# hezy18/SegMMInterest

Measured on AMD Instinct MI355X. Metric: train interactions/sec (segment-Transformer, B=512·S=40·D=768), higher is better.
Workload: dtype f32 (products via scaled fp16x2 split, 22-bit operands, fp32 accumulate; operands pre-split by their producers); 1 GPU; BASELINE config 2: synthetic SegMM B=512/GPU x S=40 x D_in=768 -> d=768, h=16, 2-layer segment encoder, image/image inputs, Lt=100 user tokens, interestBPR, dropout 0.1, AdamW; 8 distinct batches rotated; input=features; rows_per_gpu=512, global_batch=512, segments=40, feat_dim=768, in_dim=768, layers=2, parallelism=dp1, grad_allreduce_overlap=True, input_prefetch=False, delayed_scale_overflows=0, gemm_engine=f16x3p

## Files before the change

### segmminterest_amd/csrc/capi.hip

```cpp
#include <stdarg.h>
#include <stdio.h>
#include <string.h>
#include <stdlib.h>
#include <initializer_list>
#include <type_traits>

#include "../../include/segmm_hip.h"
#include "attention16.h"
#include "attention_pl.h"
#include "attention_stream.h"
#include "attention_wide.h"
#include "common.h"
#include "evalops.h"
#include "gemm.h"
#include "gemm_split.h"
#include "gemm_planes.h"
#include "gemm_planes8.h"
#include "gemm_planes4.h"
#include "loss.h"
#include "rowops.h"
#include "assemble.h"
#include "storeops.h"
#include "srops.h"

static int num_cus() {
    static int n = 0;
    if (n == 0) {
        int dev = 0;
        hipDeviceProp_t prop;
        if (hipGetDevice(&dev) == hipSuccess && hipGetDeviceProperties(&prop, dev) == hipSuccess) n = prop.multiProcessorCount;
        if (n <= 0) n = 256;
    }
    return n;
}
#ifdef SEGMM_STAMPS
static unsigned long long* g_segmm_stamps = nullptr;
extern "C" int segmm_debug_set_stamps(void* p) { g_segmm_stamps = (unsigned long long*)p; return 0; }
#endif

thread_local char g_segmm_err[512] = {0};

int segmm_fail(int code, const char* fmt, ...) {
    va_list ap;
    va_start(ap, fmt);
    vsnprintf(g_segmm_err, sizeof(g_segmm_err), fmt, ap);
    va_end(ap);
    return code;
}

#define LAUNCH_CHECK() SEGMM_CHECK_HIP(hipGetLastError())

StepState* g_segmm_step = nullptr;
static StepState* g_step_default = nullptr;
StepState* segmm_step_current() {
    if (g_segmm_step) return g_segmm_step;
    if (!g_step_default) {
        if (hipMalloc((void**)&g_step_default, sizeof(StepState)) != hipSuccess) return nullptr;
        (void)hipMemset(g_step_default, 0, sizeof(StepState));
    }
    return g_step_default;
}

using namespace segmm;

static inline int attn_keys_p(int La, int Lb) { return ((La + 15) & ~15) + ((Lb + 15) & ~15); }
static int attn_fill(AttnArgs& a, int B, int H, int dh, int Lq, int La, int Lb, const float* Qa, const float* Qb, int ldq,
                     const float* Ka, const float* Va, int ldka, const float* Kb, const float* Vb, int ldkb,
                     const uint8_t* mq, const uint8_t* mka, const uint8_t* mkb, float drop_p, uint64_t seed,
                     uint32_t site, bool planes_in = false) {
    SEGMM_REQUIRE(B > 0 && H > 0 && Lq > 0 && La >= 0 && Lb >= 0 && La + Lb > 0, "attn: empty dimension");
    if (La == 0) { Qa = Qb; Ka = Kb; Va = Vb; ldka = ldkb; mka = mkb; }
    if (Lb == 0) { Qb = Qa; Kb = Ka; Vb = Va; ldkb = ldka; mkb = mka; }
    SEGMM_REQUIRE(((Qa && Qb && Ka && Va && Kb && Vb) || (planes_in && !Qa && !Qb && !Ka && !Va && !Kb && !Vb)) && mq && mka && mkb, "attn: null pointer");
    SEGMM_REQUIRE(dh == 4 || dh == 8 || dh == 16 || dh == 32 || dh == 48 || dh == 64 || dh == 96 || dh == 128,
                  "attn: head dim %d not built (4,8,16,32,48,64,96,128)", dh);
    SEGMM_REQUIRE(!(planes_in && att_wide(dh)), "attn: input planes are not built for wide heads (head dim %d > 64): hand the fp32 views of Q / K / V", dh);
    SEGMM_REQUIRE(ldq % 4 == 0 && ldka % 4 == 0 && ldkb % 4 == 0, "attn: leading dims %% 4");
    SEGMM_REQUIRE(aligned16(Qa) && aligned16(Qb) && aligned16(Ka) && aligned16(Va) && aligned16(Kb) && aligned16(Vb), "attn: alignment");
    SEGMM_REQUIRE(Lq <= 256 && La <= 256 && Lb <= 256, "attn: Lq=%d, La=%d, Lb=%d not built (at most 256 queries and 256 keys per key block)", Lq, La, Lb);
    a.B = B; a.H = H; a.Lq = Lq; a.La = La; a.Lb = Lb;
    a.Qa = Qa; a.Qb = Qb; a.ldq = ldq; a.Ka = Ka; a.Va = Va; a.ldka = ldka; a.Kb = Kb; a.Vb = Vb; a.ldkb = ldkb;
    a.mq = mq; a.mka = mka; a.mkb = mkb;
    a.scale = 1.0f / sqrtf((float)dh);
    a.drop = make_drop(drop_p, seed, site);
    {
        const size_t ka = La ? ((size_t)B * La - 1) * ldka + (size_t)H * dh : 0, kb = Lb ? ((size_t)B * Lb - 1) * ldkb + (size_t)H * dh : 0;
        const size_t q = ((size_t)B * Lq - 1) * ldq + (size_t)H * dh;
        SEGMM_REQUIRE(((size_t)B * La + 16) * ldka * 4 < (1ull << 32) && ((size_t)B * Lb + 16) * ldkb * 4 < (1ull << 32) &&
                      ((size_t)B * Lq + 16) * ldq * 4 < (1ull << 32), "attn: a K/V/Q view exceeds the 4 GiB buffer-addressing window");
        a.ka_bytes = (uint32_t)(ka * 4); a.kb_bytes = (uint32_t)(kb * 4); a.q_bytes = (uint32_t)(q * 4);
    }
    return 0;
}

enum {
    K_ATTN, K_ATT_FWD_PL, K_ATT_FWD_LDS, K_ATT_FWD_KSPLIT, K_ATT_FWD_LDS_PAD, K_ATT_STREAM, K_ATT_FUSED_LAUNCH, K_ATT_MERGE, K_ATT_LDS_PAD, K_ATT_WAVES, K_ATT_WAVES_PL, K_ATT_REPAIR_WALK,
    K_ATT_HPB_FWD, K_ATT_HPB_DQ, K_ATT_HPB_DKV, K_L1NORM_REG, K_GEMM_BN, K_PL_VAR, K_PL_NJ, K_TN_VAR, K_LN_BWD_PARTS, K_DPRE_PLANES_ONLY, K_EMA_NT, K_LN_FWD_PARTS, K_COUNT
};
struct Knob { const char* name; int value; const char* doc; };
static Knob g_knobs[K_COUNT] = {
    {"ATTN", 1, "attention arithmetic: 0 (env: f32) exact-fp32 kernels only, 1 fp16x3 where measured faster, 2 (env: f16all) fp16x3 wherever built"},
    {"ATT_FWD_PL", 1, "planes-in forward when the caller hands input planes (0: never)"},
    {"ATT_FWD_LDS", 1, "LDS-DMA staged fp32 forward: 0 never, 1 heads with >= 4 query tiles, 2 wherever it fits"},
    {"ATT_FWD_KSPLIT", 1, "staged forward: key-tile groups per query tile"},
    {"ATT_FWD_LDS_PAD", 0, "probe: extra LDS bytes per forward workgroup (fewer workgroups per CU)"},
    {"ATT_STREAM", 0, "1: every fp32-view forward and every phase 0-3 backward through the streamed kernels (always taken above 192 padded keys)"},
    {"ATT_FUSED_LAUNCH", 2, "fused backward: 2 one launch per key block, 1 one launch for both"},
    {"ATT_MERGE", 1, "short heads: one workgroup per head for both key blocks in the fused backward"},
    {"ATT_LDS_PAD", 0, "probe: extra LDS bytes per backward workgroup"},
    {"ATT_WAVES", 4, "fused fp16x3 backward: waves per workgroup (key tiles in passes)"},
    {"ATT_WAVES_PL", 3, "planes-in fused backward: waves per workgroup, 1..4 (3: 40.7 KB of LDS -> four workgroups per CU for a 100-key block too)"},
    {"ATT_REPAIR_WALK", 512, "planes-in backward, repair launch: workgroups that walk the heads (0: one workgroup per head)"},
    {"ATT_HPB_FWD", 0, "forward workgroup shape heads | tiles << 8 (env: \"heads[,tiles]\"; 0: built-in)"},
    {"ATT_HPB_DQ", 0, "dQ kernel workgroup shape, as above"},
    {"ATT_HPB_DKV", 0, "dK/dV kernel workgroup shape, as above"},
    {"L1NORM_REG", 1, "L1 normalisation with the row held in registers"},
    {"GEMM_BN", 0, "on-the-fly GEMM: tile width override (0: built-in choice)"},
    {"PL_VAR", 4, "plane NT GEMM: 4 gemm_pl_nt4 (round 6: 128 x 256 tiles, two workgroups per CU) for K >= 768 and N >= 768, gemm_pl_nt8 otherwise; 44 gemm_pl_nt4 always; 8 gemm_pl_nt8 (round 3); 1: the round-2 fallback kernel for every launch"},
    {"PL_NJ", 0, "plane NT GEMM: tile width in 64-column units (0: modelled choice)"},
    {"TN_VAR", 8, "plane TN GEMM: 8 gemm_pl_tn4 (round 6: 128 x 256 tiles, two workgroups per CU) for few-tile and 128-row matrices, gemm_pl_tn8 (round 3) otherwise; 4 gemm_pl_tn4 wherever it fits; 88 gemm_pl_tn8 wherever it fits; 0: the round-2 fallback kernel for every launch"},
    {"LN_BWD_PARTS", 0, "LayerNorm backward: most workgroups (= partial rows of its column sums) per launch; 0: as many four-wave workgroups as are resident at the row width (768 at d = 768: one full round, no under-occupied tail)"},
    {"DPRE_PLANES_ONLY", 1, "embedding LayerNorm gradients as planes only + repair launch (no fp32 copy): 0 never, 1 for sites on the per-position grid today (rows * d >= 2^23), 2 wherever segmm_layernorm_bwd_pos_parts gives a grid (tests at small shapes), 3 as 1 for the user side only (A/B per site)"},
    {"EMA_NT", 0, "segmm_ema_update: 0 everything with the default cache policy, 1 the shadow loaded and stored nontemporally (p with the default policy); same bits (A/B: profiles/ema/)"},
    {"LN_FWD_PARTS", 0, "LayerNorm forward (d <= 1024): 0 one round of resident workgroups whose waves walk rows, grid by row width; 1 the one-wave-per-row form; 2 and up: that many workgroups in the walking form, clamped to 64..4096; same bits (A/B: profiles/row_stream/)"},
};
static bool g_knobs_ready = false;
static void knobs_init() {
    if (g_knobs_ready) return;
    g_knobs_ready = true;
    for (int k = 0; k < K_COUNT; ++k) {
        char name[64];
        snprintf(name, sizeof(name), "SEGMM_%s", g_knobs[k].name);
        const char* e = getenv(name);
        if (!e || !*e) continue;
        if (k == K_ATTN) g_knobs[k].value = !strcmp(e, "f32") ? 0 : !strcmp(e, "f16all") ? 2 : 1;
        else if (k == K_ATT_HPB_FWD || k == K_ATT_HPB_DQ || k == K_ATT_HPB_DKV) {
            const char* c = strchr(e, ',');
            g_knobs[k].value = (atoi(e) > 0 ? atoi(e) : 0) | ((c && atoi(c + 1) > 0 ? atoi(c + 1) : 0) << 8);
        } else g_knobs[k].value = atoi(e);
    }
}
static inline int knob(int k) { knobs_init(); return g_knobs[k].value; }
int segmm_config_set(const char* name, int value) {
    knobs_init();
    for (int k = 0; k < K_COUNT; ++k)
        if (!strcmp(name, g_knobs[k].name)) { const int prev = g_knobs[k].value; g_knobs[k].value = value; return prev; }
    return segmm_fail(-1, "segmm_config_set: no knob named %s (see segmm_config_dump)", name);
}
int segmm_config_dump(char* buf, int n) {
    knobs_init();
    int need = 0;
    for (int k = 0; k < K_COUNT; ++k) {
        char line[320];
        const int m = snprintf(line, sizeof(line), "SEGMM_%s=%d  # %s\n", g_knobs[k].name, g_knobs[k].value, g_knobs[k].doc);
        if (buf && need + m < n) memcpy(buf + need, line, (size_t)m + 1);
        need += m;
    }
    return need;
}

static int attn_f16() { return knob(K_ATTN); }

static void attn_shape(int n, int H, int max_waves, int want_default, int kn, int& wq, int& hpb) {
    wq = n;
    if (n > 5) {
        wq = 4;
        for (int w = 5; w >= 3; --w)
            if (n % w == 0) { wq = w; break; }
    }
    if (wq > max_waves) wq = max_waves;
    hpb = 1;
    const int e = knob(kn);
    int want = want_default;
    if (e & 0xff) {
        want = e & 0xff;
        if ((e >> 8) > 0 && (e >> 8) <= n && (e >> 8) <= max_waves) wq = e >> 8;
    }
    for (int c = want; c >= 1; --c)
        if (H % c == 0 && c * wq <= max_waves) { hpb = c; break; }
}

static bool attn_streamed(int Tp) { return Tp > 16 * 12 || knob(K_ATT_STREAM) != 0; }
template <class F>
static void attn_by_key_tiles(int Tp, F launch) {
    if (Tp <= 64) launch(std::integral_constant<int, 4>{});
    else if (Tp <= 160) launch(std::integral_constant<int, 10>{});
    else launch(std::integral_constant<int, 12>{});
}
template <int MAXW, class F>
static void attn_by_waves(int nw, F launch) {
    if (nw <= 4) launch(std::integral_constant<int, 4>{});
    else if (MAXW <= 8 || nw <= 8) launch(std::integral_constant<int, 8>{});
    else if constexpr (MAXW > 8) launch(std::integral_constant<int, 12>{});
}

template <int DH>
static bool attn_fwd_pl_takes(const AttnArgs& a) {
    if constexpr (DH % 16 != 0 || att_wide(DH)) return false;
    else {
        if (knob(K_ATT_FWD_PL) == 0) return false;
        const int nqt = (a.Lq + 15) / 16, T = a.La + a.Lb;
        return a.in.Qa && a.La % 4 == 0 && a.Lb % 4 == 0 && nqt <= ATT_PL_MAXW && T <= 16 * 12 &&
               attn_fwd_pl_lds_bytes<DH>(a.La, a.Lb) <= 160 * 1024 && (((uintptr_t)a.mka | (uintptr_t)a.mkb) & 3u) == 0;
    }
}
template <int DH>
static int attn_launch_fwd_pl(AttnArgs& a, hipStream_t s) {
// ... 288 lines not shown
        for (int i = 0; i < 8; ++i)
#pragma unroll
            for (int j = 0; j < 4; ++j)
#pragma unroll
                for (int pr = 0; pr < 3; ++pr)
                    acc[i][j] = __builtin_amdgcn_mfma_f32_16x16x32_f16(b[j], a[i], acc[i][j], 0, 0, 0);
        asm volatile("" ::: "memory");
    }
    float t = 0.f;
#pragma unroll
    for (int i = 0; i < 8; ++i)
#pragma unroll
        for (int j = 0; j < 4; ++j) t += acc[i][j].x + acc[i][j].y + acc[i][j].z + acc[i][j].w;
    if (t == 12345.678f) out[0] = t;
}
}

namespace segmm {
__global__ void step_set_kernel(StepState* st, uint32_t lo, uint32_t hi, int step, float b1, float b2) {
    st->seed_lo = lo; st->seed_hi = hi; st->step = step;
    st->bc1 = step > 0 ? (float)(1.0 - pow((double)b1, (double)step)) : 1.f;
    st->bc2_sqrt = step > 0 ? (float)sqrt(1.0 - pow((double)b2, (double)step)) : 1.f;
    st->lr = (float)segmm_lr_at(*st, step - 1);
}
__global__ void step_advance_kernel(StepState* st, float b1, float b2) {
    const int t = st->step + 1;
    st->step = t;
    const uint32_t lo = mix32(st->seed_lo + 0x9E3779B9u * (uint32_t)t);
    st->seed_hi = mix32(st->seed_hi ^ lo ^ 0x85EBCA6Bu) & 0x7fffffffu;
    st->seed_lo = lo;
    st->bc1 = (float)(1.0 - pow((double)b1, (double)t));
    st->bc2_sqrt = (float)sqrt(1.0 - pow((double)b2, (double)t));
    st->lr = (float)segmm_lr_at(*st, t - 1);
}
__global__ void step_advance_guarded_kernel(StepState* st, float b1, float b2) {
    const int t = st->step + 1;
    st->step = t;
    const uint32_t lo = mix32(st->seed_lo + 0x9E3779B9u * (uint32_t)t);
    st->seed_hi = mix32(st->seed_hi ^ lo ^ 0x85EBCA6Bu) & 0x7fffffffu;
    st->seed_lo = lo;
    const int ta = t - (int)st->skipped;
    st->bc1 = ta > 0 ? (float)(1.0 - pow((double)b1, (double)ta)) : 1.f;
    st->bc2_sqrt = ta > 0 ? (float)sqrt(1.0 - pow((double)b2, (double)ta)) : 1.f;
    st->lr = (float)segmm_lr_at(*st, t - 1);
    st->skip = 0u;
}
__global__ void step_set_skipped_kernel(StepState* st, uint32_t skipped) {
    st->skip = 0u;
    st->skipped = skipped;
}
__global__ void step_schedule_kernel(StepState* st, int kind, float base_lr, int warmup_steps, float start_factor, int decay_steps,
                                     float eta_min, float gamma, int step_size) {
    st->kind = kind; st->base_lr = base_lr; st->warmup_steps = warmup_steps; st->start_factor = start_factor;
    st->decay_steps = decay_steps; st->eta_min = eta_min; st->gamma = gamma; st->step_size = step_size;
    st->lr = (float)segmm_lr_at(*st, st->step - 1);
}
__global__ void step_base_lr_kernel(StepState* st, float base_lr) {
    st->base_lr = base_lr;
    st->lr = (float)segmm_lr_at(*st, st->step - 1);
}
}

template <class F> static void with_bools(F&& f) { f(); }
template <class F, class... Bs> static void with_bools(F&& f, bool b, Bs... bs) {
    if (b) with_bools([&](auto... cs) { f(std::true_type{}, cs...); }, bs...);
    else with_bools([&](auto... cs) { f(std::false_type{}, cs...); }, bs...);
}

extern "C" {

const char* segmm_last_error(void) { return g_segmm_err; }
int segmm_abi_version(void) { return SEGMM_ABI_VERSION; }
int segmm_attn_mode(int mode) { const int prev = attn_f16(); if (mode >= 0 && mode <= 2) g_knobs[K_ATTN].value = mode; return prev; }

static PlaneOut plane_out(uint16_t* planes, int ld2, float* hdr, const float* scale_in) {
    PlaneOut po;
    po.p = (_Float16*)planes; po.ld2 = ld2; po.hdr = hdr; po.scale_in = scale_in;
    return po;
}
#define PLANE_OUT_CHECK(what, cols)                                                                                          \
    SEGMM_REQUIRE(!planes || (hdr && (cols) % 32 == 0 && ld2 % 64 == 0 && ld2 >= 2 * (cols) && aligned16(planes)),             \
                  what ": plane output needs a header, cols %% 32, ld2 %% 64, 16-byte alignment")

int segmm_l1norm(const float* x, float* y, float* inv_scale, int64_t rows, int D, float* amax, uint16_t* planes, int ld2, float* hdr,
                 const float* scale_in, segmm_stream_t stream) {
    PLANE_OUT_CHECK("l1norm", D);
    SEGMM_REQUIRE(x && (y || inv_scale || (planes && scale_in)), "l1norm: null pointer");
    SEGMM_REQUIRE(D > 0 && D % 4 == 0 && aligned16(x) && (!y || aligned16(y)), "l1norm: D %% 4 / alignment (D=%d)", D);
    if (rows <= 0) return 0;
    const int wpb = 4;
    const int reg_form = knob(K_L1NORM_REG);
    const dim3 grid((unsigned)((rows + wpb - 1) / wpb)), block(64 * wpb);
#define L1R(V) hipLaunchKernelGGL((l1norm_reg_kernel<V>), grid, block, 0, (hipStream_t)stream, x, y, inv_scale, (long long)rows, D, amax, plane_out(planes, ld2, hdr, scale_in))
    if (reg_form && D <= 256) L1R(1);
    else if (reg_form && D <= 512) L1R(2);
    else if (reg_form && D <= 768) L1R(3);
    else if (reg_form && D <= 1024) L1R(4);
    else if (reg_form && D <= 1536) L1R(6);
    else if (reg_form && D <= 2048) L1R(8);
    else hipLaunchKernelGGL(l1norm_kernel, grid, block, 0, (hipStream_t)stream, x, y, inv_scale, (long long)rows, D, amax, plane_out(planes, ld2, hdr, scale_in));
#undef L1R
    LAUNCH_CHECK();
    return 0;
}

static inline bool aligned8(const void* p) { return (((uintptr_t)p) & 7u) == 0; }
#define ROW_H_LAUNCH(KERNEL, ...)                                                                                        \
    do {                                                                                                                 \
        if (elem == SEGMM_ELEM_F16) { ROW_H_LAUNCH_V(KERNEL, ELEM_F16, __VA_ARGS__); }                                   \
        else { ROW_H_LAUNCH_V(KERNEL, ELEM_BF16, __VA_ARGS__); }                                                         \
    } while (0)
#define ROW_H_LAUNCH_V(KERNEL, E, ...)                                                                                   \
    do {                                                                                                                 \
        if (D <= 256) hipLaunchKernelGGL((KERNEL<E, 1>), grid, block, 0, (hipStream_t)stream, __VA_ARGS__);              \
        else if (D <= 512) hipLaunchKernelGGL((KERNEL<E, 2>), grid, block, 0, (hipStream_t)stream, __VA_ARGS__);         \
        else if (D <= 768) hipLaunchKernelGGL((KERNEL<E, 3>), grid, block, 0, (hipStream_t)stream, __VA_ARGS__);         \
        else if (D <= 1024) hipLaunchKernelGGL((KERNEL<E, 4>), grid, block, 0, (hipStream_t)stream, __VA_ARGS__);        \
        else if (D <= 1536) hipLaunchKernelGGL((KERNEL<E, 6>), grid, block, 0, (hipStream_t)stream, __VA_ARGS__);        \
        else if (D <= 256 * ROW_MAXV) hipLaunchKernelGGL((KERNEL<E, 8>), grid, block, 0, (hipStream_t)stream, __VA_ARGS__); \
        else hipLaunchKernelGGL((KERNEL<E, 0>), grid, block, 0, (hipStream_t)stream, __VA_ARGS__);                       \
    } while (0)

int segmm_l1norm_h(const uint16_t* x, int elem, float* y, float* inv_scale, int64_t rows, int D, float* amax, uint16_t* planes, int ld2,
                   float* hdr, const float* scale_in, segmm_stream_t stream) {
    PLANE_OUT_CHECK("l1norm_h", D);
    SEGMM_REQUIRE(elem == SEGMM_ELEM_F16 || elem == SEGMM_ELEM_BF16, "l1norm_h: elem = %d (SEGMM_ELEM_F16 = 1, SEGMM_ELEM_BF16 = 2)", elem);
    SEGMM_REQUIRE(x && (y || inv_scale || (planes && scale_in)), "l1norm_h: null pointer");
    SEGMM_REQUIRE(D > 0 && D % 4 == 0 && aligned8(x) && (!y || aligned16(y)), "l1norm_h: D %% 4 / alignment (D=%d)", D);
    if (rows <= 0) return 0;
    const dim3 grid((unsigned)((rows + 3) / 4)), block(256);
    ROW_H_LAUNCH(l1norm_h_kernel, x, y, inv_scale, (long long)rows, D, amax, plane_out(planes, ld2, hdr, scale_in));
    LAUNCH_CHECK();
    return 0;
}

static inline bool aligned4(const void* p) { return (((uintptr_t)p) & 3u) == 0; }
static inline bool elem8(int elem) { return elem == SEGMM_ELEM_E4M3 || elem == SEGMM_ELEM_E5M2 || elem == SEGMM_ELEM_I8; }
#define ROW_B_LAUNCH(KERNEL, ...)                                                                                        \
    do {                                                                                                                 \
        if (elem == SEGMM_ELEM_E4M3) { ROW_H_LAUNCH_V(KERNEL, ELEM_E4M3, __VA_ARGS__); }                                 \
        else if (elem == SEGMM_ELEM_E5M2) { ROW_H_LAUNCH_V(KERNEL, ELEM_E5M2, __VA_ARGS__); }                            \
        else { ROW_H_LAUNCH_V(KERNEL, ELEM_I8, __VA_ARGS__); }                                                           \
    } while (0)

int segmm_l1norm_b(const uint8_t* x, int elem, float* y, float* inv_scale, int64_t rows, int D, float* amax, uint16_t* planes, int ld2,
                   float* hdr, const float* scale_in, segmm_stream_t stream) {
    PLANE_OUT_CHECK("l1norm_b", D);
    SEGMM_REQUIRE(elem8(elem), "l1norm_b: elem = %d (SEGMM_ELEM_E4M3 = 3, SEGMM_ELEM_E5M2 = 4, SEGMM_ELEM_I8 = 5)", elem);
    SEGMM_REQUIRE(x && (y || inv_scale || (planes && scale_in)), "l1norm_b: null pointer");
    SEGMM_REQUIRE(D > 0 && D % 4 == 0 && aligned4(x) && (!y || aligned16(y)), "l1norm_b: D %% 4 / alignment (D=%d)", D);
    if (rows <= 0) return 0;
    const dim3 grid((unsigned)((rows + 3) / 4)), block(256);
    ROW_B_LAUNCH(l1norm_b_kernel, x, y, inv_scale, (long long)rows, D, amax, plane_out(planes, ld2, hdr, scale_in));
    LAUNCH_CHECK();
    return 0;
}

int segmm_quantize_rows(const float* x, int64_t rows, int D, int elem, uint8_t* q, float* scale_out, segmm_stream_t stream) {
    SEGMM_REQUIRE(elem8(elem), "quantize_rows: elem = %d (SEGMM_ELEM_E4M3 = 3, SEGMM_ELEM_E5M2 = 4, SEGMM_ELEM_I8 = 5)", elem);
    SEGMM_REQUIRE(x && q && rows >= 0, "quantize_rows: null pointer / rows");
    SEGMM_REQUIRE(D > 0 && D % 4 == 0 && aligned16(x) && aligned4(q) && (!scale_out || aligned4(scale_out)),
                  "quantize_rows: D %% 4 / alignment (D=%d)", D);
    if (rows <= 0) return 0;
    const dim3 grid((unsigned)((rows + 3) / 4)), block(256);
    if (elem == SEGMM_ELEM_E4M3) hipLaunchKernelGGL((quantize_rows_kernel<ELEM_E4M3>), grid, block, 0, (hipStream_t)stream, x, (long long)rows, D, q, scale_out);
    else if (elem == SEGMM_ELEM_E5M2) hipLaunchKernelGGL((quantize_rows_kernel<ELEM_E5M2>), grid, block, 0, (hipStream_t)stream, x, (long long)rows, D, q, scale_out);
    else hipLaunchKernelGGL((quantize_rows_kernel<ELEM_I8>), grid, block, 0, (hipStream_t)stream, x, (long long)rows, D, q, scale_out);
    LAUNCH_CHECK();
    return 0;
}

static int gemm_impl(int layout, int M, int N, int K, const float* A, int lda, const float* B, int ldb, float* C, int ldc,
                     const float* bias, const float* row_scale, const float* residual, int ldr, int res_period,
                     int activation, float* aux, int ldaux, float drop_p, uint64_t seed, uint32_t site, int splits,
                     float* workspace, int accumulate, int engine, const uint16_t* a_planes, long long a_pstride,
// ... 1942 lines not shown
```

### segmminterest_amd/csrc/gemm_planes.h

```cpp
#pragma once
#include <type_traits>
#include "gemm_split.h"

namespace segmm {

struct PlaneOperand {
    const _Float16* p; int ld2;
    uint32_t bytes;
    const float* hdr;
    const float* f32; int ldf;
};
struct PGemmX {
    PlaneOperand A, B;
    _Float16* Cp; int ldc2; float* c_hdr;
    const float* c_scale_in;
    int write_c;
    int repair;
    float* colsum_out; float* colsum_ws;
    int dbg;
    unsigned long long* stamps;
};

#ifdef SEGMM_GEMM_PROBE
#define SEGMM_GEMM_DBG(q) ((q).dbg)
// ... 450 lines not shown

    const bool split = gridDim.z > 1;
    if (do_colsum && (lane & 31) == 0) {
        float* dst = split ? q.colsum_ws + (size_t)kz * p.M : q.colsum_out;
        const float inv_a = 1.f / sa;
#pragma unroll
        for (int r = 0; r < 16; ++r) {
            const int m = m0 + wm * 128 + wn * 32 + (r & 3) + 8 * (r >> 2) + 4 * (lane >> 5);
            if (m < p.M) dst[m] = (!split && p.residual) ? dst[m] + accb[r] * inv_a : accb[r] * inv_a;
        }
    }
    float* Cs = (float*)smem + wave * (32 * 64);
    const float inv_ab = (1.f / sa) * (1.f / sb);
    float* Cout = split ? p.C + (size_t)kz * (size_t)p.slab_stride : p.C;
    float am = 0.f;
#pragma unroll 1
    for (int i = 0; i < 4; ++i) {
        f32x16 c[2];
        switch (i) {
            case 0: c[0] = acc[0][0]; c[1] = acc[0][1]; break;
            case 1: c[0] = acc[1][0]; c[1] = acc[1][1]; break;
            case 2: c[0] = acc[2][0]; c[1] = acc[2][1]; break;
            default: c[0] = acc[3][0]; c[1] = acc[3][1]; break;
        }
        epi_strip_write<2>(c, Cs, lane);
        if (split) epi_strip_emit<true, 2>(p, q, Cs, lane, m0 + wm * 128 + i * 32, n0 + wn * 64, inv_ab, 0.f, Cout, am);
        else epi_strip_emit<false, 2>(p, q, Cs, lane, m0 + wm * 128 + i * 32, n0 + wn * 64, inv_ab, 0.f, Cout, am);
    }
}

__global__ __launch_bounds__(256) void split_p32_kernel(const float* __restrict__ x, long long rows, int cols, int ld,
                                                        _Float16* __restrict__ planes, int ld2, float* hdr, int mode) {
    __shared__ float red[8];
    float s;
    if (mode == 0) s = site_exact_scale(hdr, red, threadIdx.x, 256);
    else s = hdr[0];
    const int c4n = cols >> 2;
    const long long n4 = rows * c4n;
    float am = 0.f;
    bool nan = false;
    for (long long i = blockIdx.x * (long long)blockDim.x + threadIdx.x; i < n4; i += (long long)gridDim.x * blockDim.x) {
        const long long r = i / c4n;
        const int c = (int)(i - r * c4n) << 2;
        const f32x4 v = *(const f32x4*)(x + r * ld + c);
        plane_store4_pair(planes, ld2, r, c, v, s);
        am = absmax4(am, v);
        nan |= (v.x != v.x) | (v.y != v.y) | (v.z != v.z) | (v.w != v.w);
    }
    if (mode == 0) {
        if (blockIdx.x == 0 && threadIdx.x == 0) { hdr[0] = s; hdr[1] = 0.f; }
    } else {
        site_commit(hdr, am, blockIdx.x * 4 + (threadIdx.x >> 6), s);
        if (nan && s > 0.f) ((volatile unsigned int*)hdr)[1] = 1u;
    }
}
__global__ __launch_bounds__(256) void split_p32_transpose_kernel(const float* __restrict__ x, int R, int Cc, int ld,
                                                                  _Float16* __restrict__ planes, int ld2, const float* hdr) {
    __shared__ float tile[32][33];
    const float s = hdr[0];
    const int r0 = blockIdx.y * 32, c0 = blockIdx.x * 32;
    const int tx = threadIdx.x & 31, ty = threadIdx.x >> 5;
#pragma unroll
    for (int k = 0; k < 4; ++k) {
        const int r = r0 + ty + 8 * k, c = c0 + tx;
        tile[ty + 8 * k][tx] = (r < R && c < Cc) ? x[(size_t)r * ld + c] : 0.f;
    }
    __syncthreads();
#pragma unroll
    for (int k = 0; k < 4; ++k) {
        const int c = c0 + ty + 8 * k, r = r0 + tx;
        if (c < Cc && r < R) {
            const float v = tile[tx][ty + 8 * k];
            const _Float16 h = (_Float16)__builtin_fmaf(v, s, 0.f);
            const _Float16 l = (_Float16)__builtin_fmaf(v, s, -(float)h);
            _Float16* o = planes + (size_t)c * ld2 + ((r >> 5) << 6) + (r & 31);
            o[0] = h; o[32] = l;
        }
    }
}

struct WMat { long long off; int R, Cc, tr, tile0, tcols; };
__global__ __launch_bounds__(256) void wabsmax_kernel(const float* __restrict__ flat, const WMat* __restrict__ desc, float* hdr) {
    const WMat m = desc[blockIdx.y];
    const float* x = flat + m.off;
    const long long n4 = (long long)m.R * m.Cc / 4;
    float am = 0.f;
    for (long long i = blockIdx.x * (long long)blockDim.x + threadIdx.x; i < n4; i += (long long)gridDim.x * blockDim.x)
        am = absmax4(am, *(const f32x4*)(x + 4 * i));
    am = wave_max(am);
    if ((threadIdx.x & 63) == 0) hdr[(size_t)blockIdx.y * SITE_FLOATS + SITE_HDR + blockIdx.x * 4 + (threadIdx.x >> 6)] = am;
}
__global__ __launch_bounds__(256) void wsplit_kernel(const float* __restrict__ flat, const WMat* __restrict__ desc, int n_mats, float* hdr,
                                                     _Float16* __restrict__ wpl, _Float16* __restrict__ wTpl) {
    __shared__ float tile[32][33];
    __shared__ float red[8];
    int mi = 0;
    while (mi + 1 < n_mats && (int)blockIdx.x >= desc[mi + 1].tile0) ++mi;
    const WMat m = desc[mi];
    float* h = hdr + (size_t)mi * SITE_FLOATS;
    const float s = site_exact_scale(h, red, threadIdx.x, 256);
    const int t = blockIdx.x - m.tile0;
    const int r0 = (t / m.tcols) * 32, c0 = (t % m.tcols) * 32;
    if (t == 0 && threadIdx.x == 0) { h[0] = s; h[1] = 0.f; }
    const float* x = flat + m.off;
    const int tx = threadIdx.x & 31, ty = threadIdx.x >> 5;
#pragma unroll
    for (int k = 0; k < 4; ++k) {
        const int r = r0 + ty + 8 * k, c = c0 + tx;
        const float v = (r < m.R && c < m.Cc) ? x[(size_t)r * m.Cc + c] : 0.f;
        tile[ty + 8 * k][tx] = v;
        if (r < m.R && c < m.Cc) {
            const _Float16 hi = (_Float16)__builtin_fmaf(v, s, 0.f);
            const _Float16 lo = (_Float16)__builtin_fmaf(v, s, -(float)hi);
            _Float16* o = wpl + 2 * m.off + (size_t)r * (2 * m.Cc) + ((c >> 5) << 6) + (c & 31);
            o[0] = hi; o[32] = lo;
        }
    }
    if (!m.tr) return;
    __syncthreads();
#pragma unroll
    for (int k = 0; k < 4; ++k) {
        const int c = c0 + ty + 8 * k, r = r0 + tx;
        if (c < m.Cc && r < m.R) {
            const float v = tile[tx][ty + 8 * k];
            const _Float16 hi = (_Float16)__builtin_fmaf(v, s, 0.f);
            const _Float16 lo = (_Float16)__builtin_fmaf(v, s, -(float)hi);
            _Float16* o = wTpl + 2 * m.off + (size_t)c * (2 * m.R) + ((r >> 5) << 6) + (r & 31);
            o[0] = hi; o[32] = lo;
        }
    }
}

}
```

### segmminterest_amd/csrc/rowops.h

```cpp
#pragma once
#include "common.h"

namespace segmm {
constexpr int ROW_MAXV = 8;

__global__ __launch_bounds__(256) void l1norm_kernel(const float* __restrict__ x, float* y, float* inv_scale, long long rows, int D,
                                                     float* amax, PlaneOut po) {
    const int lane = threadIdx.x & 63;
    const long long row = (long long)blockIdx.x * (blockDim.x >> 6) + (threadIdx.x >> 6);
    if (row >= rows) return;
    const float* xr = x + row * D;
    float s = 0.f;
    for (int c = lane * 4; c < D; c += 256) {
        const f32x4 v = *(const f32x4*)(xr + c);
        s += fabsf(v.x) + fabsf(v.y) + fabsf(v.z) + fabsf(v.w);
    }
    s = wave_sum(s);
    const float inv = 1.0f / (s + 1e-6f);
    if (inv_scale && lane == 0) inv_scale[row] = inv;
    const float ps = plane_scale(po);
    if (y || ps > 0.f) {
        const float den = s + 1e-6f;
        float am = 0.f;
        for (int c = lane * 4; c < D; c += 256) {
            f32x4 v = *(const f32x4*)(xr + c);
            v.x /= den; v.y /= den; v.z /= den; v.w /= den;
            if (y) *(f32x4*)(y + row * D + c) = v;
            if (ps > 0.f) plane_store4_pair(po.p, po.ld2, row, c, v, ps);
            am = absmax4(am, v);
        }
        plane_finish(po, amax, am, (unsigned)row, ps, row == 0 && lane == 0);
    }
}

template <int V>
__global__ __launch_bounds__(256) void l1norm_reg_kernel(const float* __restrict__ x, float* y, float* inv_scale, long long rows, int D,
                                                         float* amax, PlaneOut po) {
    const int lane = threadIdx.x & 63;
    const long long row = (long long)blockIdx.x * (blockDim.x >> 6) + (threadIdx.x >> 6);
    if (row >= rows) return;
    const float* xr = x + row * D;
    f32x4 v[V];
    float s = 0.f;
#pragma unroll
    for (int i = 0; i < V; ++i) {
        const int c = lane * 4 + i * 256;
        v[i] = f32x4{0.f, 0.f, 0.f, 0.f};
        if (c < D) { v[i] = ld_row4b(xr + c); s += fabsf(v[i].x) + fabsf(v[i].y) + fabsf(v[i].z) + fabsf(v[i].w); }
    }
    s = wave_sum(s);
    const float inv = 1.0f / (s + 1e-6f);
    if (inv_scale && lane == 0) inv_scale[row] = inv;
    const float ps = plane_scale(po);
    if (y || ps > 0.f) {
        const float den = s + 1e-6f;
        float am = 0.f;
#pragma unroll
        for (int i = 0; i < V; ++i) {
            const int c = lane * 4 + i * 256;
            if (c < D) {
                f32x4 o = v[i];
                o.x /= den; o.y /= den; o.z /= den; o.w /= den;
                if (y) st_row4b(y + row * D + c, o);
                if (ps > 0.f) plane_store4_pair(po.p, po.ld2, row, c, o, ps);
                am = absmax4(am, o);
            }
        }
        plane_finish(po, amax, am, (unsigned)row, ps, row == 0 && lane == 0);
    }
}

template <int ELEM, int V>
__global__ __launch_bounds__(256) void l1norm_h_kernel(const uint16_t* __restrict__ x, float* y, float* inv_scale, long long rows, int D,
                                                       float* amax, PlaneOut po) {
    const int lane = threadIdx.x & 63;
    const long long row = (long long)blockIdx.x * (blockDim.x >> 6) + (threadIdx.x >> 6);
    if (row >= rows) return;
    const uint16_t* xr = x + row * D;
    uint32_t ra[V > 0 ? V : 1], rb[V > 0 ? V : 1];
    float s = 0.f;
    if constexpr (V > 0) {
#pragma unroll
        for (int i = 0; i < V; ++i) {
            const int c = lane * 4 + i * 256;
            ra[i] = rb[i] = 0u;
            if (c < D) {
                const u32x2 w = ld_row4h(xr + c);
                ra[i] = w.x; rb[i] = w.y;
                const f32x4 v = widen4<ELEM>(ra[i], rb[i]);
                s += fabsf(v.x) + fabsf(v.y) + fabsf(v.z) + fabsf(v.w);
            }
        }
    } else {
        for (int c = lane * 4; c < D; c += 256) {
            const f32x4 v = widen4<ELEM>(ld_row4h(xr + c));
            s += fabsf(v.x) + fabsf(v.y) + fabsf(v.z) + fabsf(v.w);
        }
    }
    s = wave_sum(s);
    const float inv = 1.0f / (s + 1e-6f);
    if (inv_scale && lane == 0) inv_scale[row] = inv;
    const float ps = plane_scale(po);
    if (y || ps > 0.f) {
        const float den = s + 1e-6f;
        float am = 0.f;
        if constexpr (V > 0) {
#pragma unroll
            for (int i = 0; i < V; ++i) {
                const int c = lane * 4 + i * 256;
                if (c < D) {
                    f32x4 o = widen4<ELEM>(ra[i], rb[i]);
                    o.x /= den; o.y /= den; o.z /= den; o.w /= den;
                    if (y) st_row4b(y + row * D + c, o);
                    if (ps > 0.f) plane_store4_pair(po.p, po.ld2, row, c, o, ps);
                    am = absmax4(am, o);
                }
            }
        } else {
            for (int c = lane * 4; c < D; c += 256) {
                f32x4 o = widen4<ELEM>(ld_row4h(xr + c));
                o.x /= den; o.y /= den; o.z /= den; o.w /= den;
                if (y) *(f32x4*)(y + row * D + c) = o;
                if (ps > 0.f) plane_store4_pair(po.p, po.ld2, row, c, o, ps);
                am = absmax4(am, o);
            }
        }
        plane_finish(po, amax, am, (unsigned)row, ps, row == 0 && lane == 0);
    }
}

template <int ELEM, int V>
__global__ __launch_bounds__(256) void l1norm_b_kernel(const uint8_t* __restrict__ x, float* y, float* inv_scale, long long rows, int D,
                                                       float* amax, PlaneOut po) {
    const int lane = threadIdx.x & 63;
    const long long row = (long long)blockIdx.x * (blockDim.x >> 6) + (threadIdx.x >> 6);
    if (row >= rows) return;
    const uint8_t* xr = x + row * D;
    uint32_t rw[V > 0 ? V : 1];
    float s = 0.f;
    if constexpr (V > 0) {
#pragma unroll
        for (int i = 0; i < V; ++i) {
            const int c = lane * 4 + i * 256;
            rw[i] = 0u;
            if (c < D) {
                rw[i] = ld_row4q(xr + c);
                const f32x4 v = widen4<ELEM>(rw[i]);
                s += fabsf(v.x) + fabsf(v.y) + fabsf(v.z) + fabsf(v.w);
            }
        }
    } else {
        for (int c = lane * 4; c < D; c += 256) {
// ... 1129 lines not shown
```

Measured before the change: 144,100 interactions/s.

## Add row-walking L1 norm kernel and vectorise weight absmax/split kernels

Adds a persistent row-walking L1 normalisation kernel that prefetches the next row into registers and merges amax writes into one slot per wave when the stride allows, selected by default through a new knob. Separately, the weight absmax kernel is unrolled eight-deep to keep more loads in flight. The weight split kernel now uses a binary search for its matrix, float4 loads, f16x4 stores, and a packed hi/lo LDS transpose. These target memory latency and narrow stores in small per-step kernels, at the cost of more code paths and a new amax slot-merging rule.

Result: no change. 143,900 interactions/s (-0.1%).

```diff
diff --git a/segmminterest_amd/csrc/capi.hip b/segmminterest_amd/csrc/capi.hip
--- a/segmminterest_amd/csrc/capi.hip
+++ b/segmminterest_amd/csrc/capi.hip
@@ -95,7 +95,7 @@
 
 enum {
     K_ATTN, K_ATT_FWD_PL, K_ATT_FWD_LDS, K_ATT_FWD_KSPLIT, K_ATT_FWD_LDS_PAD, K_ATT_STREAM, K_ATT_FUSED_LAUNCH, K_ATT_MERGE, K_ATT_LDS_PAD, K_ATT_WAVES, K_ATT_WAVES_PL, K_ATT_REPAIR_WALK,
-    K_ATT_HPB_FWD, K_ATT_HPB_DQ, K_ATT_HPB_DKV, K_L1NORM_REG, K_GEMM_BN, K_PL_VAR, K_PL_NJ, K_TN_VAR, K_LN_BWD_PARTS, K_DPRE_PLANES_ONLY, K_EMA_NT, K_LN_FWD_PARTS, K_COUNT
+    K_ATT_HPB_FWD, K_ATT_HPB_DQ, K_ATT_HPB_DKV, K_L1NORM_REG, K_GEMM_BN, K_PL_VAR, K_PL_NJ, K_TN_VAR, K_LN_BWD_PARTS, K_DPRE_PLANES_ONLY, K_EMA_NT, K_LN_FWD_PARTS, K_L1NORM_PARTS, K_COUNT
 };
 struct Knob { const char* name; int value; const char* doc; };
 static Knob g_knobs[K_COUNT] = {
@@ -123,6 +123,7 @@
     {"DPRE_PLANES_ONLY", 1, "embedding LayerNorm gradients as planes only + repair launch (no fp32 copy): 0 never, 1 for sites on the per-position grid today (rows * d >= 2^23), 2 wherever segmm_layernorm_bwd_pos_parts gives a grid (tests at small shapes), 3 as 1 for the user side only (A/B per site)"},
     {"EMA_NT", 0, "segmm_ema_update: 0 everything with the default cache policy, 1 the shadow loaded and stored nontemporally (p with the default policy); same bits (A/B: profiles/ema/)"},
     {"LN_FWD_PARTS", 0, "LayerNorm forward (d <= 1024): 0 one round of resident workgroups whose waves walk rows, grid by row width; 1 the one-wave-per-row form; 2 and up: that many workgroups in the walking form, clamped to 64..4096; same bits (A/B: profiles/row_stream/)"},
+    {"L1NORM_PARTS", 0, "L1 normalisation, fp32 rows (D <= 1024, L1NORM_REG on): 0 one round of resident workgroups whose waves walk rows; 1 the one-wave-per-row form; 2 and up: that many workgroups in the walking form, clamped to 64..4096; same bits (A/B: profiles/step_head/)"},
 };
 static bool g_knobs_ready = false;
 static void knobs_init() {
@@ -577,6 +578,13 @@
     SEGMM_REQUIRE(!planes || (hdr && (cols) % 32 == 0 && ld2 % 64 == 0 && ld2 >= 2 * (cols) && aligned16(planes)),             \
                   what ": plane output needs a header, cols %% 32, ld2 %% 64, 16-byte alignment")
 
+static int l1norm_cap(int D) {
+    const int k = knob(K_L1NORM_PARTS);
+    if (k == 1 || D > 1024) return 0;
+    if (k >= 2) return k < 64 ? 64 : k > 4096 ? 4096 : k;
+    return D <= 768 ? 2048 : 1536;
+}
+
 int segmm_l1norm(const float* x, float* y, float* inv_scale, int64_t rows, int D, float* amax, uint16_t* planes, int ld2, float* hdr,
                  const float* scale_in, segmm_stream_t stream) {
     PLANE_OUT_CHECK("l1norm", D);
@@ -585,7 +593,18 @@
     if (rows <= 0) return 0;
     const int wpb = 4;
     const int reg_form = knob(K_L1NORM_REG);
-    const dim3 grid((unsigned)((rows + wpb - 1) / wpb)), block(64 * wpb);
+    const dim3 block(64 * wpb);
+    const int64_t per_row = (rows + wpb - 1) / wpb;
+    const int cap = reg_form ? l1norm_cap(D) : 0;
+    if (cap > 0) {
+        const dim3 grid((unsigned)(per_row < cap ? per_row : cap));
+#define L1W(V) hipLaunchKernelGGL((l1norm_walk_kernel<V>), grid, block, 0, (hipStream_t)stream, x, y, inv_scale, (long long)rows, D, amax, plane_out(planes, ld2, hdr, scale_in))
+        if (D <= 256) L1W(1); else if (D <= 512) L1W(2); else if (D <= 768) L1W(3); else L1W(4);
+#undef L1W
+        LAUNCH_CHECK();
+        return 0;
+    }
+    const dim3 grid((unsigned)per_row);
 #define L1R(V) hipLaunchKernelGGL((l1norm_reg_kernel<V>), grid, block, 0, (hipStream_t)stream, x, y, inv_scale, (long long)rows, D, amax, plane_out(planes, ld2, hdr, scale_in))
     if (reg_form && D <= 256) L1R(1);
     else if (reg_form && D <= 512) L1R(2);
diff --git a/segmminterest_amd/csrc/gemm_planes.h b/segmminterest_amd/csrc/gemm_planes.h
--- a/segmminterest_amd/csrc/gemm_planes.h
+++ b/segmminterest_amd/csrc/gemm_planes.h
@@ -556,53 +556,85 @@
 struct WMat { long long off; int R, Cc, tr, tile0, tcols; };
 __global__ __launch_bounds__(256) void wabsmax_kernel(const float* __restrict__ flat, const WMat* __restrict__ desc, float* hdr) {
     const WMat m = desc[blockIdx.y];
-    const float* x = flat + m.off;
+    const f32x4* x4 = (const f32x4*)(flat + m.off);
     const long long n4 = (long long)m.R * m.Cc / 4;
+    const long long st = (long long)gridDim.x * blockDim.x;
     float am = 0.f;
-    for (long long i = blockIdx.x * (long long)blockDim.x + threadIdx.x; i < n4; i += (long long)gridDim.x * blockDim.x)
-        am = absmax4(am, *(const f32x4*)(x + 4 * i));
+    long long i = blockIdx.x * (long long)blockDim.x + threadIdx.x;
+    for (; i + 7 * st < n4; i += 8 * st) {
+        f32x4 v[8];
+#pragma unroll
+        for (int k = 0; k < 8; ++k) v[k] = x4[i + k * st];
+#pragma unroll
+        for (int k = 0; k < 8; ++k) am = absmax4(am, v[k]);
+    }
+    if (i < n4) {
+        f32x4 v[7];
+#pragma unroll
+        for (int k = 0; k < 7; ++k) v[k] = i + k * st < n4 ? x4[i + k * st] : f32x4{0.f, 0.f, 0.f, 0.f};
+#pragma unroll
+        for (int k = 0; k < 7; ++k) am = absmax4(am, v[k]);
+    }
     am = wave_max(am);
     if ((threadIdx.x & 63) == 0) hdr[(size_t)blockIdx.y * SITE_FLOATS + SITE_HDR + blockIdx.x * 4 + (threadIdx.x >> 6)] = am;
 }
+typedef _Float16 f16x4 __attribute__((ext_vector_type(4)));
 __global__ __launch_bounds__(256) void wsplit_kernel(const float* __restrict__ flat, const WMat* __restrict__ desc, int n_mats, float* hdr,
                                                      _Float16* __restrict__ wpl, _Float16* __restrict__ wTpl) {
-    __shared__ float tile[32][33];
-    __shared__ float red[8];
-    int mi = 0;
-    while (mi + 1 < n_mats && (int)blockIdx.x >= desc[mi + 1].tile0) ++mi;
+    __shared__ uint32_t tile[32][33];
+    int mi = 0, last = n_mats - 1;
+    while (mi < last) {
+        const int mid = (mi + last + 1) >> 1;
+        if ((int)blockIdx.x >= desc[mid].tile0) mi = mid; else last = mid - 1;
+    }
     const WMat m = desc[mi];
     float* h = hdr + (size_t)mi * SITE_FLOATS;
-    const float s = site_exact_scale(h, red, threadIdx.x, 256);
     const int t = blockIdx.x - m.tile0;
     const int r0 = (t / m.tcols) * 32, c0 = (t % m.tcols) * 32;
-    if (t == 0 && threadIdx.x == 0) { h[0] = s; h[1] = 0.f; }
     const float* x = flat + m.off;
-    const int tx = threadIdx.x & 31, ty = threadIdx.x >> 5;
-#pragma unroll
-    for (int k = 0; k < 4; ++k) {
-        const int r = r0 + ty + 8 * k, c = c0 + tx;
-        const float v = (r < m.R && c < m.Cc) ? x[(size_t)r * m.Cc + c] : 0.f;
-        tile[ty + 8 * k][tx] = v;
-        if (r < m.R && c < m.Cc) {
-            const _Float16 hi = (_Float16)__builtin_fmaf(v, s, 0.f);
-            const _Float16 lo = (_Float16)__builtin_fmaf(v, s, -(float)hi);
+    const int ty = threadIdx.x >> 3, tx = (threadIdx.x & 7) << 2;
+    {
+        const int r = r0 + ty, c = c0 + tx;
+        const bool inside = r < m.R && c < m.Cc;
+        f32x4 v = {0.f, 0.f, 0.f, 0.f};
+        if (inside) v = *(const f32x4*)(x + (size_t)r * m.Cc + c);
+        const float s = f16_scale_of(site_amax(h, threadIdx.x & 63));
+        if (t == 0 && threadIdx.x == 0) { h[0] = s; h[1] = 0.f; }
+        if (inside) {
+            f16x4 hi, lo;
+#pragma unroll
+            for (int k = 0; k < 4; ++k) {
+                hi[k] = (_Float16)__builtin_fmaf(v[k], s, 0.f);
+                lo[k] = (_Float16)__builtin_fmaf(v[k], s, -(float)hi[k]);
+            }
             _Float16* o = wpl + 2 * m.off + (size_t)r * (2 * m.Cc) + ((c >> 5) << 6) + (c & 31);
-            o[0] = hi; o[32] = lo;
+            *(f16x4*)o = hi;
+            *(f16x4*)(o + 32) = lo;
+            if (m.tr) {
+                const uint2 hb = __builtin_bit_cast(uint2, hi), lb = __builtin_bit_cast(uint2, lo);
+                tile[ty][tx + 0] = (hb.x & 0xffffu) | (lb.x << 16);
+                tile[ty][tx + 1] = (hb.x >> 16) | (lb.x & 0xffff0000u);
+                tile[ty][tx + 2] = (hb.y & 0xffffu) | (lb.y << 16);
+                tile[ty][tx + 3] = (hb.y >> 16) | (lb.y & 0xffff0000u);
+            }
         }
     }
     if (!m.tr) return;
     __syncthreads();
-#pragma unroll
-    for (int k = 0; k < 4; ++k) {
-        const int c = c0 + ty + 8 * k, r = r0 + tx;
-        if (c < m.Cc && r < m.R) {
-            const float v = tile[tx][ty + 8 * k];
-            const _Float16 hi = (_Float16)__builtin_fmaf(v, s, 0.f);
-            const _Float16 lo = (_Float16)__builtin_fmaf(v, s, -(float)hi);
-            _Float16* o = wTpl + 2 * m.off + (size_t)c * (2 * m.R) + ((r >> 5) << 6) + (r & 31);
-            o[0] = hi; o[32] = lo;
-        }
-    }
-}
-
-}
+    const int c = c0 + ty, r = r0 + tx;
+    if (c >= m.Cc || r >= m.R) return;
+    _Float16* o = wTpl + 2 * m.off + (size_t)c * (2 * m.R) + ((r >> 5) << 6) + (r & 31);
+    if ((m.R & 3) == 0) {
+        const uint32_t e0 = tile[tx + 0][ty], e1 = tile[tx + 1][ty], e2 = tile[tx + 2][ty], e3 = tile[tx + 3][ty];
+        *(uint2*)o = make_uint2((e0 & 0xffffu) | (e1 << 16), (e2 & 0xffffu) | (e3 << 16));
+        *(uint2*)(o + 32) = make_uint2((e0 >> 16) | (e1 & 0xffff0000u), (e2 >> 16) | (e3 & 0xffff0000u));
+    } else {
+        uint16_t* o16 = (uint16_t*)o;
+        for (int k = 0; k < 4 && r + k < m.R; ++k) {
+            const uint32_t e = tile[tx + k][ty];
+            o16[k] = (uint16_t)e; o16[k + 32] = (uint16_t)(e >> 16);
+        }
+    }
+}
+
+}
diff --git a/segmminterest_amd/csrc/rowops.h b/segmminterest_amd/csrc/rowops.h
--- a/segmminterest_amd/csrc/rowops.h
+++ b/segmminterest_amd/csrc/rowops.h
@@ -68,6 +68,64 @@
         }
         plane_finish(po, amax, am, (unsigned)row, ps, row == 0 && lane == 0);
     }
+}
+
+template <int V>
+__global__ __launch_bounds__(256) void l1norm_walk_kernel(const float* __restrict__ x, float* y, float* inv_scale, long long rows, int D,
+                                                          float* amax, PlaneOut po) {
+    const int lane = threadIdx.x & 63;
+    const long long stride = (long long)gridDim.x * (blockDim.x >> 6);
+    long long row = (long long)blockIdx.x * (blockDim.x >> 6) + (threadIdx.x >> 6);
+    if (row >= rows) return;
+    f32x4 nx[V];
+#pragma unroll
+    for (int i = 0; i < V; ++i) {
+        const int c = lane * 4 + i * 256;
+        nx[i] = f32x4{0.f, 0.f, 0.f, 0.f};
+        if (c < D) nx[i] = ld_row4b(x + row * D + c);
+    }
+    const float ps = plane_scale(po);
+    const bool normalise = y || ps > 0.f;
+    const bool one_slot = (stride & (AMAX_SLOTS - 1)) == 0 || row + stride >= rows;
+    const long long row0 = row;
+    float am = 0.f;
+    for (; row < rows; row += stride) {
+        f32x4 v[V];
+        float s = 0.f;
+#pragma unroll
+        for (int i = 0; i < V; ++i) {
+            const int c = lane * 4 + i * 256;
+            v[i] = nx[i];
+            if (c < D) s += fabsf(v[i].x) + fabsf(v[i].y) + fabsf(v[i].z) + fabsf(v[i].w);
+        }
+        if (row + stride < rows) {
+#pragma unroll
+            for (int i = 0; i < V; ++i) {
+                const int c = lane * 4 + i * 256;
+                if (c < D) nx[i] = ld_row4b(x + (row + stride) * D + c);
+            }
+        }
+        s = wave_sum(s);
+        const float inv = 1.0f / (s + 1e-6f);
+        if (inv_scale && lane == 0) inv_scale[row] = inv;
+        if (normalise) {
+            const float den = s + 1e-6f;
+            if (!one_slot) am = 0.f;
+#pragma unroll
+            for (int i = 0; i < V; ++i) {
+                const int c = lane * 4 + i * 256;
+                if (c < D) {
+                    f32x4 o = v[i];
+                    o.x /= den; o.y /= den; o.z /= den; o.w /= den;
+                    if (y) st_row4b(y + row * D + c, o);
+                    if (ps > 0.f) plane_store4_pair(po.p, po.ld2, row, c, o, ps);
+                    am = absmax4(am, o);
+                }
+            }
+            if (!one_slot) plane_finish(po, amax, am, (unsigned)row, ps, row == 0 && lane == 0);
+        }
+    }
+    if (normalise && one_slot) plane_finish(po, amax, am, (unsigned)row0, ps, row0 == 0 && lane == 0);
 }
 
 template <int ELEM, int V>
```
